# mathisbot/homomorph-rust

Measured on AMD Instinct MI355X. Metric: homomorphic u32 ops/sec (add, mul) at d=dp=tau=128; 1/2/4/8 MI355X, higher is better.
Workload: dtype u32

## Files before the change

### homomorph-rust_amd/csrc/adder_mfma.hip

```cpp
#include <hip/hip_runtime.h>

#include "mfma_gf2.h"

namespace hm {

#ifdef HM_MFMA_PROFILE
__device__ unsigned long long *g_mfma_prof;
#define HM_PT(v) const unsigned long long v = __builtin_amdgcn_s_memtime()
#define HM_PACC(k, a, b) prof[k] += (b) - (a)
#else
#define HM_PT(v)
#define HM_PACC(k, a, b)
#endif

#ifndef HM_MFMA_PREFETCH
#define HM_MFMA_PREFETCH 3
#endif
#ifndef HM_MFMA_PREFETCH25
#define HM_MFMA_PREFETCH25 4
#endif
template <int NC> constexpr int kPrefetchOf = NC > 16 ? HM_MFMA_PREFETCH25 : NC <= 8 ? 2 : HM_MFMA_PREFETCH;
template <int NC> constexpr int kStage(int k) { return NC <= 8 ? 2 * k : 1 + 3 * k; }
template <int NC, class Side, int kPrefetch = kPrefetchOf<NC>>
__device__ __forceinline__ v16f tile_mfma(const v8i (&Af)[NC], const uint4 *rb, const uint4 *rbn,
                                          uint4 (&pf)[kPrefetch], v16f acc, Side &&side) {
    static_assert(NC - kPrefetch > kStage<NC>(2), "next tile's B reads must follow its ring fill (stage 2)");
    uint4 bq[NC];
#pragma unroll
    for (int c = 0; c < kPrefetch; ++c) bq[c] = pf[c];
#pragma unroll
    for (int c = 0; c < NC; ++c) {
        if (c + kPrefetch < NC) bq[c + kPrefetch] = rb[2 * (c + kPrefetch)];
        else pf[c + kPrefetch - NC] = rbn[2 * (c + kPrefetch - NC)];
        const v8i Bf = {(int)bq[c].x, (int)bq[c].y, (int)bq[c].z, (int)bq[c].w, 0, 0, 0, 0};
        acc = mfma_fp4(Af[c], Bf, acc);
        asm volatile("" : "+v"(acc)::"memory");
        if (c == kStage<NC>(0)) side(0);
        if (c == kStage<NC>(1)) side(1);
        if (c == kStage<NC>(2)) side(2);
    }
    return acc;
}

template <int kMirror>
__device__ __forceinline__ void ring_put(uint32_t *ring, int w, int h, uint2 nb) {
    const int s = w & (kMfmaRingSlots - 1);
    uint32_t *slot = &ring[s * 4 + 2 * h];
    *(uint2 *)slot = nb;
    if (kMirror >= kMfmaRingSlots || s < kMirror) *(uint2 *)(slot + 4 * kMfmaRingSlots) = nb;
}

#ifndef HM_RING_PAIRS
#define HM_RING_PAIRS 1
#endif
template <int kMirror>
__device__ __forceinline__ void ring_fill(const uint32_t *C, uint32_t *ring, const uint32_t *tab,
                                          int base, int count, int lane) {
    const int h = HM_RING_PAIRS ? lane & 1 : lane >> 5;
    for (int k = HM_RING_PAIRS ? lane >> 1 : lane & 31; k < count; k += 32) {
        const int w = base + k;
        const uint32_t v = C[w] >> (16 * h);
        uint2 nb;
        nb.x = tab[v & 0xFFu];
        nb.y = tab[(v >> 8) & 0xFFu];
        ring_put<kMirror>(ring, w, h, nb);
    }
}

#ifndef HM_REC_WAIT_YOUNG
#define HM_REC_WAIT_YOUNG 0
#endif
__device__ __forceinline__ void wait_record(int young) {
    if (!HM_REC_WAIT_YOUNG || young <= 0) asm volatile("s_waitcnt vmcnt(0)" ::: "memory");
    else if (young >= 16) asm volatile("s_waitcnt vmcnt(16)" ::: "memory");
    else if (young >= 8) asm volatile("s_waitcnt vmcnt(8)" ::: "memory");
    else if (young >= 4) asm volatile("s_waitcnt vmcnt(4)" ::: "memory");
    else if (young >= 2) asm volatile("s_waitcnt vmcnt(2)" ::: "memory");
    else asm volatile("s_waitcnt vmcnt(1)" ::: "memory");
}

#ifndef HM_MFMA_WPB
#define HM_MFMA_WPB kAddWavesPerBlock
#endif
constexpr int kMfmaWpb = HM_MFMA_WPB;
static_assert(kMfmaWpb <= kAddWavesPerBlock, "host LDS plan");

template <int NC>
__global__ void __launch_bounds__(64 * kMfmaWpb)
__attribute__((amdgpu_waves_per_eu(MfmaCfg<NC>::kWavesPerEU, MfmaCfg<NC>::kWavesPerEU)))
add_chain_mfma_kernel(AddArgs A) {
    kt_start(A.kt);
    using Cfg = MfmaCfg<NC>;
    constexpr int kRevWords = Cfg::kRevWords, kRsWords = Cfg::kRsWords, kRec = Cfg::kRecWords;
    extern __shared__ uint32_t lds[];
    __shared__ uint32_t stage[kMfmaWpb][2][kRec];
    uint32_t *tab = lds;
    for (uint32_t k = threadIdx.x; k < 256; k += blockDim.x) {
        uint32_t v = 0u;
#pragma unroll
        for (int t = 0; t < 8; ++t) v |= ((k >> t) & 1u) << (4 * t + 1);
        tab[k] = v;
    }
    __syncthreads();
    const int wave = (int)rfl(threadIdx.x >> 6);
    const uint64_t e = (uint64_t)blockIdx.x * (blockDim.x >> 6) + wave;
    if (e >= A.n) {
        kt_finish(A.kt);
        return;
    }
    const int lane = lane_id();
    const uint32_t L = A.nbits;
    uint32_t *Ls = lds + 256 + (size_t)wave * A.chain_lds;
    uint32_t *C = Ls + Cfg::kHalo;
    uint32_t *ring = C + A.mf_cw;
    uint32_t *RS = ring + Cfg::kRingWords;
    const uint32_t *ws = A.ws + e * A.ws_stride;
    uint64_t *po = A.out.limbs + e * A.out.stride;
    uint32_t *dout = A.out.degree + e * L;
    const uint32_t oP = A.cntX, oAB = oP + A.cntP, oD = oAB + A.cntAB;
    auto rec_word = [&](uint32_t u, uint32_t &base, uint32_t &step) {
        const uint32_t offD = L * (A.cntAB + A.cntP);
        if (u < oP) base = offD + 2 * L + u, step = A.cntX;
        else if (u < oAB) base = L * A.cntAB + (u - oP), step = A.cntP;
        else if (u < oD) base = u - oAB, step = A.cntAB;
        else if (u == oD + 1) base = offD, step = 1;
        else base = offD + L, step = 1;
    };
    uint32_t lbase, lstep, lbase2 = 0, lstep2 = 0;
    rec_word((uint32_t)lane, lbase, lstep);
    if constexpr (kRec > 64) rec_word(64u + (uint32_t)lane, lbase2, lstep2);
    const bool two = kRec > 64 && oD + 2 > 64;
    const uint64_t wsu = ((uint64_t)rfl((uint32_t)((uintptr_t)ws >> 32)) << 32) |
                         rfl((uint32_t)(uintptr_t)ws);
    auto stage_rec = [&](uint32_t i) {
        const uint32_t voff = 4u * (lbase + i * lstep);
        const uint32_t m0 = (uint32_t)(uintptr_t)&stage[wave][i & 1][0];
        asm volatile("s_mov_b32 m0, %2\n\ts_nop 0\n\tglobal_load_lds_dword %0, %1"
                     :
                     : "v"(voff), "s"(wsu), "s"(m0)
                     : "memory", "m0");
        if (two) {
            const uint32_t voff2 = 4u * (lbase2 + i * lstep2);
            asm volatile("s_mov_b32 m0, %2\n\ts_nop 0\n\tglobal_load_lds_dword %0, %1"
                         :
                         : "v"(voff2), "s"(wsu), "s"(m0 + 256u)
                         : "memory", "m0");
        }
    };
    stage_rec(0);

#ifdef HM_MFMA_PROFILE
    unsigned long long prof[4] = {0, 0, 0, 0};
#endif
    for (uint32_t k = lane; k < Cfg::kHalo + A.mf_cw; k += kWave) Ls[k] = 0u;
    for (int k = 4 * kRevWords + lane; k < kRsWords; k += kWave) RS[k] = 0u;
    wsync();
    int nc = 0;
    int degc = -1;
    int tw = -1;
    int young = 0;
    uint32_t offo = 0;
    for (uint32_t i = 0; i < L; ++i) {
        HM_PT(tw0);
        wait_record(young);
        young = 0;
        const uint32_t *rec = &stage[wave][i & 1][0];
        HM_PT(t0);
        HM_PACC(3, tw0, t0);
        if (tw < 0) {
            store_sum_x(rec, (int)A.cntX, C, nc, po + offo, A.ob.b[i], dout + i, A.status);
        } else {
            const int capw = 2 * (int)cap_of(A.ob.b[i]);
            uint32_t *so = (uint32_t *)(po + offo);
            int ldeg = -1;
            if (lane < 32) {
                const uint32_t v = (lane < (int)A.cntX ? rec[lane] : 0u) ^ C[lane];
                if (lane < capw) so[lane] = v;
                if (v) ldeg = lane * 32 + 31 - (int)__builtin_clz(v);
            }
            for (int w = tw + lane; w < capw; w += kWave) so[w] = 0u;
            int deg = wave_max_i32(ldeg);
            if (nc > 32) deg = degc;
            if (lane == 0) {
                if (deg > (int)A.ob.b[i]) flag(A.status, HM_ERR_CAPACITY);
                dout[i] = (uint32_t)max(deg, 0);
            }
        }
        offo += cap_of(A.ob.b[i]);
        HM_PT(t1);
        HM_PACC(0, t0, t1);
        if (i + 1 == L) break;
        const int np = bitwords((int)rfl(rec[oD])), nab = bitwords((int)rfl(rec[oD + 1]));
        const uint32_t *abi = rec + oAB;
        wsync();
        if (np == 0 || nc == 0) {
            const int n = max(nc, nab);
            for (int w = lane; w < n; w += kWave) C[w] = w < nab ? abi[w] : 0u;
            nc = nab;
            degc = (int)rfl(rec[oD + 1]) - 1;
            tw = -1;
            wsync();
            stage_rec(i + 1);
            continue;
        }
        const uint32_t *pi = rec + oP;
        for (int k = lane; k < 4 * kRevWords; k += kWave) {
            const int q = kRevWords - 1 - (k >> 2);
            const uint32_t rev = __builtin_bitreverse32(q < np ? pi[q] : 0u);
            RS[k] = tab[(rev >> (8 * (k & 3))) & 0xFFu];
        }
        wsync();
        stage_rec(i + 1);
        const int D = np;
        const int lane = lane_opaque(), col = lane & 31, h = lane >> 5;
        v8i Af[NC];
        const int jb = 32 * (kRevWords - D + h) - 1 - row_bit(col);
        const uint32_t *rw0 = RS + (jb >> 3);
        const uint32_t sh = 4u * (uint32_t)(jb & 7);
#pragma unroll
        for (int c = 0; c < NC; ++c) {
            const uint32_t *rw = rw0 + 8 * c;
            const uint32_t w0 = rw[0], w1 = rw[1], w2 = rw[2], w3 = rw[3], w4 = rw[4];
            Af[c] = (v8i){(int)funnel(w1, w0, sh), (int)funnel(w2, w1, sh), (int)funnel(w3, w2, sh),
                          (int)funnel(w4, w3, sh), 0, 0, 0, 0};
        }
        HM_PT(t2);
        HM_PACC(1, t1, t2);
        const int nout = max(nc + np, nab);
        const int tiles = (nout + 31) >> 5;
        uint32_t *son = (uint32_t *)(po + offo);
        const int capn = 2 * (int)cap_of(A.ob.b[i + 1]);
        const int wlo = 32;
        ring_fill<Cfg::kMirror>(C, ring, tab, 32 * (tiles - 1) - D, 32 + 2 * NC, lane);
        int ldeg = -1;
        const int alg = (int)rfl(rec[oD]) - 1 + degc;
        const bool track = alg <= (int)rfl(rec[oD + 1]) - 1;
        v16f acc;
#pragma unroll
        for (int j = 0; j < 16; ++j) acc[j] = 8388608.0f;
        uint32_t gprev = 0u;
        auto rbase = [&](int T) {
            return (const uint4 *)&ring[((32 * T + col - D + h) & (kMfmaRingSlots - 1)) * 4];
        };
        wsync();
        constexpr int kPrefetch = kPrefetchOf<NC>;
        uint4 pf[kPrefetch];
#pragma unroll
        for (int c = 0; c < kPrefetch; ++c) pf[c] = rbase(tiles - 1)[2 * c];
        const uint4 *rb = rbase(tiles - 1);
        for (int T = tiles - 1; T >= 0; --T) {
            wsync();
            if constexpr (NC > 16) rb = rbase(T);
            const uint4 *rbn = rbase(T - 1);
            const int fh = HM_RING_PAIRS ? lane & 1 : h;
            const int fw = 32 * (T - 1) - D + (HM_RING_PAIRS ? lane >> 1 : col);
            uint32_t fv;
            uint2 fn;
            const int W = 32 * T + col;
            uint32_t abw = 0u;
            if (32 * T < nab) {
                asm volatile("" ::: "memory");
                abw = W < nab ? abi[W] : 0u;
            }
            __builtin_amdgcn_s_setprio(1);
            acc = tile_mfma<NC>(Af, rb, rbn, pf, acc, [&](int stage) {
                if (stage == 0) fv = C[fw];
                else if (stage == 1) {
                    asm volatile("" : "+v"(fv));
                    fv >>= 16 * fh;
                    fn.x = tab[fv & 0xFFu], fn.y = tab[(fv >> 8) & 0xFFu];
                } else {
                    asm volatile("" : "+v"(fn.x), "+v"(fn.y));
                    ring_put<Cfg::kMirror>(ring, fw, fh, fn);
                }
            });
            __builtin_amdgcn_s_setprio(0);
            const uint32_t tnow = acc_parities_hi16(acc);
            const uint32_t t = (tnow ^ gprev) >> (16 - 16 * h);
            const auto sw = __builtin_amdgcn_permlane32_swap(t, gprev, false, false);
            gprev = tnow;
            const uint32_t word = sw[0] | sw[1];
            const uint32_t v = word ^ abw;
            const bool full = T >= 1 && 32 * T + 32 <= capn;
            young += full ? 1 : 0;
            if (h == 0) {
                C[W] = v;
                if (full) {
                    asm volatile("" ::: "memory");
                    son[W] = v;
                } else if (W >= wlo && W < capn) son[W] = v;
            }
            if (track) {
                asm volatile("" ::: "memory");
                int Wq = W;
                asm volatile("" : "+v"(Wq));
                if (h == 0 && v) ldeg = max(ldeg, Wq * 32 + 31 - (int)__builtin_clz(v));
            }
            rb = rbn;
        }
        const int deg = track ? wave_max_i32(ldeg) : alg;
        nc = deg >= 0 ? (deg >> 5) + 1 : 0;
        degc = deg;
        tw = 32 * tiles;
        wsync();
        HM_PT(t3);
        HM_PACC(2, t2, t3);
    }
#ifdef HM_MFMA_PROFILE
    if (lane == 0)
        for (int k = 0; k < 4; ++k) g_mfma_prof[e * 4 + k] = prof[k];
#endif
    kt_finish(A.kt);
}

int launch_add_chain_mfma(const AddArgs &a, void *stream) {
    const int wpb = kMfmaWpb;
    const uint64_t blocks = (a.n + wpb - 1) / wpb;
    const size_t lds = (256 + (size_t)a.chain_lds * wpb) * 4;
#define HM_LAUNCH_CHAIN(NCV)                                                                      \
    hipLaunchKernelGGL((add_chain_mfma_kernel<NCV>), dim3((unsigned)blocks), dim3(64 * wpb), lds,  \
                       (hipStream_t)stream, a)
    if (a.mfma == MfmaCfg<7>::kChunks) HM_LAUNCH_CHAIN(7);
    else if (a.mfma == MfmaCfg<13>::kChunks) HM_LAUNCH_CHAIN(13);
    else if (a.mfma == MfmaCfg<25>::kChunks) HM_LAUNCH_CHAIN(25);
    else return -1;
#undef HM_LAUNCH_CHAIN
    return hipGetLastError() == hipSuccess ? 0 : -1;
}

}
```

### homomorph-rust_amd/csrc/mfma_gf2.h

```cpp
#pragma once
#include <hip/hip_runtime.h>

#include "dev_common.h"

namespace hm {

typedef int v8i __attribute__((ext_vector_type(8)));
typedef float v16f __attribute__((ext_vector_type(16)));

__device__ __forceinline__ v16f mfma_fp4(const v8i &a, const v8i &b, const v16f &c) {
    return __builtin_amdgcn_mfma_scale_f32_32x32x64_f8f6f4(a, b, c, 4, 4, 0, 127, 0, 127);
}

__device__ __forceinline__ int lane_opaque() {
    int l;
    asm volatile("v_mbcnt_lo_u32_b32 %0, -1, 0\n\tv_mbcnt_hi_u32_b32 %0, -1, %0" : "=v"(l));
    return l;
}

__device__ __forceinline__ void nibble_table(uint32_t *tab) {
    for (uint32_t k = threadIdx.x; k < 256; k += blockDim.x) {
        uint32_t v = 0u;
#pragma unroll
        for (int t = 0; t < 8; ++t) v |= ((k >> t) & 1u) << (4 * t + 1);
        tab[k] = v;
    }
}

__device__ __forceinline__ v8i a_fragment(const uint32_t *rw, uint32_t sh) {
    const uint32_t w0 = rw[0], w1 = rw[1], w2 = rw[2], w3 = rw[3], w4 = rw[4];
    return (v8i){(int)funnel(w1, w0, sh), (int)funnel(w2, w1, sh), (int)funnel(w3, w2, sh),
                 (int)funnel(w4, w3, sh), 0, 0, 0, 0};
}

__device__ __forceinline__ v8i b_fragment(const uint4 &q) {
    return (v8i){(int)q.x, (int)q.y, (int)q.z, (int)q.w, 0, 0, 0, 0};
}

__host__ __device__ constexpr int row_bit(int m) { return (m & 3) + 4 * (m >> 3) + 16 * ((m >> 2) & 1); }
__device__ __forceinline__ uint32_t acc_parities_hi16(const v16f &acc) {
    uint32_t x = __float_as_uint(acc[0]) << 31;
#pragma unroll
    for (int j = 1; j < 16; ++j) x = funnel(__float_as_uint(acc[j]), x, 1);
    return x;
}

__device__ __forceinline__ uint32_t join_halves(uint32_t t_shifted) {
    const auto sw = __builtin_amdgcn_permlane32_swap(t_shifted, t_shifted, false, false);
    return sw[0] | sw[1];
}

}
```

Measured before the change: 8.819 million.

## Use explicit LDS address arithmetic and a four-phase ring in MFMA adder

Replaces generic pointers into the ring, RS and C with 32-bit LDS addresses held in opaque registers. The modulo ring indexing becomes a four-phase ring with a rolling per-tile offset, and the byte-wise ring fill reads nibble bytes directly from C instead of shift-and-mask. Global sum stores use inline SGPR-base global_store_dword, and W is recomputed from the lane id to cut live VGPRs. The aim is fewer address-calculation instructions and less register pressure in the hot tile loop. The risk is correctness: the four-phase ring must stay consistent with kMfmaRingSlots and the mirror layout.

```diff
diff --git a/homomorph-rust_amd/csrc/adder_mfma.hip b/homomorph-rust_amd/csrc/adder_mfma.hip
--- a/homomorph-rust_amd/csrc/adder_mfma.hip
+++ b/homomorph-rust_amd/csrc/adder_mfma.hip
@@ -22,16 +22,16 @@
 template <int NC> constexpr int kPrefetchOf = NC > 16 ? HM_MFMA_PREFETCH25 : NC <= 8 ? 2 : HM_MFMA_PREFETCH;
 template <int NC> constexpr int kStage(int k) { return NC <= 8 ? 2 * k : 1 + 3 * k; }
 template <int NC, class Side, int kPrefetch = kPrefetchOf<NC>>
-__device__ __forceinline__ v16f tile_mfma(const v8i (&Af)[NC], const uint4 *rb, const uint4 *rbn,
-                                          uint4 (&pf)[kPrefetch], v16f acc, Side &&side) {
+__device__ __forceinline__ v16f tile_mfma(const v8i (&Af)[NC], uint32_t rb, uint32_t rbn,
+                                          u32x4 (&pf)[kPrefetch], v16f acc, Side &&side) {
     static_assert(NC - kPrefetch > kStage<NC>(2), "next tile's B reads must follow its ring fill (stage 2)");
-    uint4 bq[NC];
+    u32x4 bq[NC];
 #pragma unroll
     for (int c = 0; c < kPrefetch; ++c) bq[c] = pf[c];
 #pragma unroll
     for (int c = 0; c < NC; ++c) {
-        if (c + kPrefetch < NC) bq[c + kPrefetch] = rb[2 * (c + kPrefetch)];
-        else pf[c + kPrefetch - NC] = rbn[2 * (c + kPrefetch - NC)];
+        if (c + kPrefetch < NC) bq[c + kPrefetch] = lds_at<const u32x4>(rb)[2 * (c + kPrefetch)];
+        else pf[c + kPrefetch - NC] = lds_at<const u32x4>(rbn)[2 * (c + kPrefetch - NC)];
         const v8i Bf = {(int)bq[c].x, (int)bq[c].y, (int)bq[c].z, (int)bq[c].w, 0, 0, 0, 0};
         acc = mfma_fp4(Af[c], Bf, acc);
         asm volatile("" : "+v"(acc)::"memory");
@@ -42,30 +42,7 @@
     return acc;
 }
 
-template <int kMirror>
-__device__ __forceinline__ void ring_put(uint32_t *ring, int w, int h, uint2 nb) {
-    const int s = w & (kMfmaRingSlots - 1);
-    uint32_t *slot = &ring[s * 4 + 2 * h];
-    *(uint2 *)slot = nb;
-    if (kMirror >= kMfmaRingSlots || s < kMirror) *(uint2 *)(slot + 4 * kMfmaRingSlots) = nb;
-}
-
-#ifndef HM_RING_PAIRS
-#define HM_RING_PAIRS 1
-#endif
-template <int kMirror>
-__device__ __forceinline__ void ring_fill(const uint32_t *C, uint32_t *ring, const uint32_t *tab,
-                                          int base, int count, int lane) {
-    const int h = HM_RING_PAIRS ? lane & 1 : lane >> 5;
-    for (int k = HM_RING_PAIRS ? lane >> 1 : lane & 31; k < count; k += 32) {
-        const int w = base + k;
-        const uint32_t v = C[w] >> (16 * h);
-        uint2 nb;
-        nb.x = tab[v & 0xFFu];
-        nb.y = tab[(v >> 8) & 0xFFu];
-        ring_put<kMirror>(ring, w, h, nb);
-    }
-}
+constexpr uint32_t kPhaseBytes = 16u * 32u;
 
 #ifndef HM_REC_WAIT_YOUNG
 #define HM_REC_WAIT_YOUNG 0
@@ -77,6 +54,10 @@
     else if (young >= 4) asm volatile("s_waitcnt vmcnt(4)" ::: "memory");
     else if (young >= 2) asm volatile("s_waitcnt vmcnt(2)" ::: "memory");
     else asm volatile("s_waitcnt vmcnt(1)" ::: "memory");
+}
+
+__device__ __forceinline__ void sum_store(uint64_t base, uint32_t off, uint32_t v) {
+    asm volatile("global_store_dword %0, %1, %2" : : "v"(off), "v"(v), "s"(base) : "memory");
 }
 
 #ifndef HM_MFMA_WPB
@@ -215,11 +196,11 @@
         const int lane = lane_opaque(), col = lane & 31, h = lane >> 5;
         v8i Af[NC];
         const int jb = 32 * (kRevWords - D + h) - 1 - row_bit(col);
-        const uint32_t *rw0 = RS + (jb >> 3);
+        const uint32_t rw0 = lds_opaque(lds_addr(RS) + 4u * (uint32_t)(jb >> 3));
         const uint32_t sh = 4u * (uint32_t)(jb & 7);
 #pragma unroll
         for (int c = 0; c < NC; ++c) {
-            const uint32_t *rw = rw0 + 8 * c;
+            const HM_LDS uint32_t *rw = lds_at<const uint32_t>(rw0) + 8 * c;
             const uint32_t w0 = rw[0], w1 = rw[1], w2 = rw[2], w3 = rw[3], w4 = rw[4];
             Af[c] = (v8i){(int)funnel(w1, w0, sh), (int)funnel(w2, w1, sh), (int)funnel(w3, w2, sh),
                           (int)funnel(w4, w3, sh), 0, 0, 0, 0};
@@ -228,10 +209,10 @@
         HM_PACC(1, t1, t2);
         const int nout = max(nc + np, nab);
         const int tiles = (nout + 31) >> 5;
-        uint32_t *son = (uint32_t *)(po + offo);
+        const uint64_t sonv = (uint64_t)(uintptr_t)(po + offo);
+        const uint64_t son = ((uint64_t)rfl((uint32_t)(sonv >> 32)) << 32) | rfl((uint32_t)sonv);
         const int capn = 2 * (int)cap_of(A.ob.b[i + 1]);
         const int wlo = 32;
-        ring_fill<Cfg::kMirror>(C, ring, tab, 32 * (tiles - 1) - D, 32 + 2 * NC, lane);
         int ldeg = -1;
         const int alg = (int)rfl(rec[oD]) - 1 + degc;
         const bool track = alg <= (int)rfl(rec[oD + 1]) - 1;
@@ -239,39 +220,63 @@
 #pragma unroll
         for (int j = 0; j < 16; ++j) acc[j] = 8388608.0f;
         uint32_t gprev = 0u;
-        auto rbase = [&](int T) {
-            return (const uint4 *)&ring[((32 * T + col - D + h) & (kMfmaRingSlots - 1)) * 4];
-        };
+        const uint32_t rb0 = lds_opaque(lds_addr(ring) + 16u * (uint32_t)(col + h));
+        const uint32_t put0 = lds_opaque(lds_addr(ring) + 8u * (uint32_t)lane);
+        uint32_t cF = lds_opaque(lds_addr(C) + 4u * (uint32_t)(32 * (tiles - 2) - D + (lane >> 1)) +
+                                 2u * (uint32_t)(lane & 1));
+        uint32_t cW = lds_opaque(lds_addr(C) + 4u * (uint32_t)(32 * (tiles - 1) + col));
+        const uint32_t col4 = 4u * (uint32_t)col;
+        auto rbase = [&](int T) { return rb0 + kPhaseBytes * (uint32_t)(T & 3); };
+        {
+            constexpr int kPasses = (32 + 2 * NC + 31) / 32;
+            uint32_t f0[kPasses], f1[kPasses];
+#pragma unroll
+            for (int p = 0; p < kPasses; ++p) {
+                f0[p] = lds_at<const uint8_t>(cF)[128 * (p + 1)];
+                f1[p] = lds_at<const uint8_t>(cF)[128 * (p + 1) + 1];
+            }
+#pragma unroll
+            for (int p = 0; p < kPasses; ++p) f0[p] = tab[f0[p]], f1[p] = tab[f1[p]];
+#pragma unroll
+            for (int p = 0; p < kPasses; ++p) {
+                const uint32_t ph = kPhaseBytes * (uint32_t)((tiles - 1 + p) & 3);
+                const u32x2 fn = {f0[p], f1[p]};
+                *lds_at<u32x2>(put0 + ph) = fn;
+                if (ph < 16u * (uint32_t)Cfg::kMirror) *lds_at<u32x2>(put0 + ph + 16u * kMfmaRingSlots) = fn;
+            }
+        }
         wsync();
         constexpr int kPrefetch = kPrefetchOf<NC>;
-        uint4 pf[kPrefetch];
-#pragma unroll
-        for (int c = 0; c < kPrefetch; ++c) pf[c] = rbase(tiles - 1)[2 * c];
-        const uint4 *rb = rbase(tiles - 1);
+        u32x4 pf[kPrefetch];
+#pragma unroll
+        for (int c = 0; c < kPrefetch; ++c) pf[c] = lds_at<const u32x4>(rbase(tiles - 1))[2 * c];
+        uint32_t rb = rbase(tiles - 1);
+        uint32_t abw = 0u;
         for (int T = tiles - 1; T >= 0; --T) {
             wsync();
             if constexpr (NC > 16) rb = rbase(T);
-            const uint4 *rbn = rbase(T - 1);
-            const int fh = HM_RING_PAIRS ? lane & 1 : h;
-            const int fw = 32 * (T - 1) - D + (HM_RING_PAIRS ? lane >> 1 : col);
-            uint32_t fv;
-            uint2 fn;
-            const int W = 32 * T + col;
-            uint32_t abw = 0u;
+            const uint32_t ph = kPhaseBytes * (uint32_t)((T - 1) & 3);
+            const uint32_t rbn = rb0 + ph;
+            const uint32_t pp = put0 + ph;
+            const bool mirror = ph < 16u * (uint32_t)Cfg::kMirror;
+            uint32_t f0, f1;
+            u32x2 fn;
             if (32 * T < nab) {
                 asm volatile("" ::: "memory");
+                const int W = 32 * T + (lane_opaque() & 31);
                 abw = W < nab ? abi[W] : 0u;
             }
             __builtin_amdgcn_s_setprio(1);
             acc = tile_mfma<NC>(Af, rb, rbn, pf, acc, [&](int stage) {
-                if (stage == 0) fv = C[fw];
-                else if (stage == 1) {
-                    asm volatile("" : "+v"(fv));
-                    fv >>= 16 * fh;
-                    fn.x = tab[fv & 0xFFu], fn.y = tab[(fv >> 8) & 0xFFu];
+                if (stage == 0) {
+                    f0 = lds_at<const uint8_t>(cF)[0], f1 = lds_at<const uint8_t>(cF)[1];
+                } else if (stage == 1) {
+                    asm volatile("" : "+v"(f0), "+v"(f1));
+                    fn.x = tab[f0], fn.y = tab[f1];
                 } else {
-                    asm volatile("" : "+v"(fn.x), "+v"(fn.y));
-                    ring_put<Cfg::kMirror>(ring, fw, fh, fn);
+                    asm volatile("" : "+v"(fn));
+                    *lds_at<u32x2>(pp) = fn;
+                    if (mirror) *lds_at<u32x2>(pp + 16u * kMfmaRingSlots) = fn;
                 }
             });
             __builtin_amdgcn_s_setprio(0);
@@ -284,19 +289,23 @@
             const bool full = T >= 1 && 32 * T + 32 <= capn;
             young += full ? 1 : 0;
             if (h == 0) {
-                C[W] = v;
+                *lds_at<uint32_t>(cW) = v;
+                const uint64_t sT = son + 128u * (uint32_t)T;
                 if (full) {
-                    asm volatile("" ::: "memory");
-                    son[W] = v;
-                } else if (W >= wlo && W < capn) son[W] = v;
+                    sum_store(sT, col4, v);
+                } else {
+                    const int W = 32 * T + (lane_opaque() & 31);
+                    if (W >= wlo && W < capn) sum_store(sT, col4, v);
+                }
             }
             if (track) {
                 asm volatile("" ::: "memory");
-                int Wq = W;
-                asm volatile("" : "+v"(Wq));
+                const int Wq = 32 * T + (lane_opaque() & 31);
                 if (h == 0 && v) ldeg = max(ldeg, Wq * 32 + 31 - (int)__builtin_clz(v));
             }
             rb = rbn;
+            cF -= 128u;
+            cW -= 128u;
         }
         const int deg = track ? wave_max_i32(ldeg) : alg;
         nc = deg >= 0 ? (deg >> 5) + 1 : 0;
diff --git a/homomorph-rust_amd/csrc/mfma_gf2.h b/homomorph-rust_amd/csrc/mfma_gf2.h
--- a/homomorph-rust_amd/csrc/mfma_gf2.h
+++ b/homomorph-rust_amd/csrc/mfma_gf2.h
@@ -17,6 +17,16 @@
     asm volatile("v_mbcnt_lo_u32_b32 %0, -1, 0\n\tv_mbcnt_hi_u32_b32 %0, -1, %0" : "=v"(l));
     return l;
 }
+
+typedef uint32_t u32x2 __attribute__((ext_vector_type(2)));
+typedef uint32_t u32x4 __attribute__((ext_vector_type(4)));
+#define HM_LDS __attribute__((address_space(3)))
+__device__ __forceinline__ uint32_t lds_addr(const void *p) { return (uint32_t)(uintptr_t)p; }
+__device__ __forceinline__ uint32_t lds_opaque(uint32_t a) {
+    asm volatile("" : "+v"(a));
+    return a;
+}
+template <class T> __device__ __forceinline__ HM_LDS T *lds_at(uint32_t a) { return (HM_LDS T *)a; }
 
 __device__ __forceinline__ void nibble_table(uint32_t *tab) {
     for (uint32_t k = threadIdx.x; k < 256; k += blockDim.x) {
```

Measured after the change: 9.239 million (median of 6 runs). +4.8%, better.
